# tooHotSpot/FGN

Hardware: AMD Instinct MI355X
Metric: query-imgs/sec (3-way 3-shot, 800x1333 FGN simple_test) (higher is better)
Workload: dtype f32; 1 GPU; cfg3: COCO2VOC 3-way 3-shot, query 3x800x1333, supports 9x3x256^2, ResNet-50-C4, R<=300 proposals, D<=100 detections, 1 episode(s) per GPU per step; h2d_in_step=True, gt_mask_rle_in_step=True, world_size_seen=1, phase_lock=rpn, caller_streams=2, support_cache=False, hip_graph=True, winograd_3x3=F(4x4,3x3)

## Files before the change

### fgn_amd/csrc/spatial.hip

```cpp
#include "common.h"

__global__ void nchw3_to_nhwc4_kernel(const float* __restrict__ x, float4* __restrict__ y, int HW,
                                      long long total) {
    for (long long i = blockIdx.x * (long long)blockDim.x + threadIdx.x; i < total;
         i += (long long)gridDim.x * blockDim.x) {
        const long long b = i / HW;
        const int p = (int)(i - b * HW);
        const float* s = x + b * 3 * HW + p;
        y[i] = make_float4(s[0], s[HW], s[2 * (size_t)HW], 0.f);
    }
}

extern "C" int fgn_nchw3_to_nhwc4_f32(const float* x, float* y, int n_img, int H, int W,
                                      hipStream_t stream) {
    if (!x || !y) return FGN_ERR_ARG;
    const long long total = (long long)n_img * H * W;
    if (total == 0) return FGN_OK;
    const int grid = (int)std::min<long long>((total + 255) / 256, 256 * 8);
    hipLaunchKernelGGL(nchw3_to_nhwc4_kernel, dim3(grid), dim3(256), 0, stream, x,
                       reinterpret_cast<float4*>(y), H * W, total);
    FGN_LAUNCH_CHECK();
    return FGN_OK;
}

// ... 155 lines not shown
    if (!src || !dst) return FGN_ERR_ARG;
    if (G < 0 || h < 0 || w < 0 || H < 0 || W < 0 || h > RESIZE_MAX_DIM || w > RESIZE_MAX_DIM || H > RESIZE_MAX_DIM ||
        W > RESIZE_MAX_DIM)
        return FGN_ERR_SHAPE;
    if ((long long)G * H * W == 0) return FGN_OK;
    if (h == 0 || w == 0) return FGN_ERR_SHAPE;
    const int chunks = cdiv(W + 3, 256);
    const long long units = (long long)G * H * chunks;
    if (units > INT32_MAX - 16 * RESIZE_GRID_CAP) return FGN_ERR_SHAPE;
    const int grid = (int)std::min<long long>((units + RESIZE_BLOCK / 64 - 1) / (RESIZE_BLOCK / 64), RESIZE_GRID_CAP * 4);
    hipLaunchKernelGGL(resize_mask_u8_kernel, dim3(grid), dim3(RESIZE_BLOCK), 0, stream, src, dst, h, w, H, W, chunks,
                       (int)units);
    FGN_LAUNCH_CHECK();
    return FGN_OK;
}

__global__ void maxpool3x3s2_kernel(const float4* __restrict__ x, float4* __restrict__ y, int H, int W,
                                    int C4, int Ho, int Wo, long long total) {
    for (long long i = blockIdx.x * (long long)blockDim.x + threadIdx.x; i < total;
         i += (long long)gridDim.x * blockDim.x) {
        const int c = (int)(i % C4);
        long long r = i / C4;
        const int ox = (int)(r % Wo);
        r /= Wo;
        const int oy = (int)(r % Ho);
        const long long b = r / Ho;
        float4 m = make_float4(-INFINITY, -INFINITY, -INFINITY, -INFINITY);
#pragma unroll
        for (int ky = 0; ky < 3; ++ky) {
            const int iy = oy * 2 - 1 + ky;
            if ((unsigned)iy >= (unsigned)H) continue;
#pragma unroll
            for (int kx = 0; kx < 3; ++kx) {
                const int ix = ox * 2 - 1 + kx;
                if ((unsigned)ix >= (unsigned)W) continue;
                const float4 v = x[((b * H + iy) * W + ix) * C4 + c];
                m.x = fmaxf(m.x, v.x); m.y = fmaxf(m.y, v.y);
                m.z = fmaxf(m.z, v.z); m.w = fmaxf(m.w, v.w);
            }
        }
        y[i] = m;
    }
}

extern "C" int fgn_maxpool3x3s2_nhwc_f32(const float* x, float* y, int n_img, int H, int W, int C,
                                         hipStream_t stream) {
    if (!x || !y) return FGN_ERR_ARG;
    if (C % 4) return FGN_ERR_SHAPE;
    const int Ho = (H + 2 - 3) / 2 + 1, Wo = (W + 2 - 3) / 2 + 1;
    const long long total = (long long)n_img * Ho * Wo * (C / 4);
    if (total == 0) return FGN_OK;
    const int grid = (int)std::min<long long>((total + 255) / 256, 256 * 16);
    hipLaunchKernelGGL(maxpool3x3s2_kernel, dim3(grid), dim3(256), 0, stream,
                       reinterpret_cast<const float4*>(x), reinterpret_cast<float4*>(y), H, W, C / 4, Ho,
                       Wo, total);
    FGN_LAUNCH_CHECK();
    return FGN_OK;
}

struct AxisSample {
    int lo, hi;
    float l, h;
    bool valid;
};

__device__ __forceinline__ AxisSample axis_sample(float c, int size) {
    AxisSample s;
    s.valid = !(c < -1.0f || c > (float)size);
    if (c <= 0.f) c = 0.f;
    int lo = (int)c;
    int hi;
    if (lo >= size - 1) {
        hi = lo = size - 1;
        c = (float)lo;
    } else {
        hi = lo + 1;
    }
    s.lo = lo; s.hi = hi;
    s.l = c - (float)lo;
    s.h = 1.f - s.l;
    return s;
}

__global__ __launch_bounds__(256) void roi_align_kernel(const float* __restrict__ fmap,
                                                        const float* __restrict__ rois,
                                                        float* __restrict__ out,
                                                        const int32_t* __restrict__ n_rois_dev, int n_rois,
                                                        int H, int W, int C, int P, float spatial_scale,
                                                        int sampling_ratio, int aligned,
                                                        const float* __restrict__ post_shift, int relu,
                                                        const float* __restrict__ fmap2, float* __restrict__ out2, int C2,
                                                        const float* __restrict__ post_shift2, int relu2) {
    const int bin = blockIdx.x;
    const int r = bin / (P * P);
    int nr = n_rois;
    if (n_rois_dev) nr = min(nr, *n_rois_dev);
    if (r >= nr) return;
    const int pb = bin - r * P * P;
    const int ph = pb / P, pw = pb - ph * P;

    const float* roi = rois + (size_t)r * 5;
    const int b = (int)roi[0];
    const float off = aligned ? 0.5f : 0.f;
    const float x1 = roi[1] * spatial_scale - off;
    const float y1 = roi[2] * spatial_scale - off;
    const float x2 = roi[3] * spatial_scale - off;
    const float y2 = roi[4] * spatial_scale - off;
    float rw = x2 - x1, rh = y2 - y1;
    if (!aligned) {
        rw = fmaxf(rw, 1.f);
        rh = fmaxf(rh, 1.f);
    }
    const float bin_h = rh / (float)P, bin_w = rw / (float)P;
    const int gh = sampling_ratio > 0 ? sampling_ratio : (int)ceilf(rh / (float)P);
    const int gw = sampling_ratio > 0 ? sampling_ratio : (int)ceilf(rw / (float)P);
    const float count = (float)max(gh * gw, 1);
    const float* base1 = fmap + (size_t)b * H * W * C;
    const float* base2 = fmap2 ? fmap2 + (size_t)b * H * W * C2 : nullptr;
    const int c_all = C + (fmap2 ? C2 : 0);
    const int C1 = C;

    constexpr int MAXS = 32;
    __shared__ float wy_sh[MAXS], wx_sh[MAXS];
    __shared__ int span_sh[4];
    if (threadIdx.x < 2) {
        const bool is_y = threadIdx.x == 0;
        const int g = is_y ? gh : gw, size = is_y ? H : W;
        const float start = (is_y ? y1 + (float)ph * bin_h : x1 + (float)pw * bin_w), step = is_y ? bin_h : bin_w;
        float* w = is_y ? wy_sh : wx_sh;
        int first = 0, last = -1;
        if (g > 0) {
            const AxisSample s0 = axis_sample(start + 0.5f * step / (float)g, size);
            const AxisSample s1 = axis_sample(start + ((float)(g - 1) + 0.5f) * step / (float)g, size);
            first = min(s0.lo, s1.lo);
            last = max(s0.hi, s1.hi);
        }
        const int n = last - first + 1;
        span_sh[is_y ? 0 : 2] = first;
        span_sh[is_y ? 1 : 3] = n;
        if (n <= MAXS) {
            for (int i = 0; i < n; ++i) w[i] = 0.f;
            for (int i = 0; i < g; ++i) {
                const AxisSample sp = axis_sample(start + ((float)i + 0.5f) * step / (float)g, size);
                if (sp.valid) {
                    w[sp.lo - first] += sp.h;
                    w[sp.hi - first] += sp.l;
                }
            }
        }
    }
    __syncthreads();
    const int y0 = span_sh[0], ny = span_sh[1], x0 = span_sh[2], nx = span_sh[3];
    const bool separable = ny <= MAXS && nx <= MAXS;

    for (int cc = threadIdx.x * 4; cc < c_all; cc += blockDim.x * 4) {
        const bool snd = cc >= C1;
        const float* base = snd ? base2 : base1;
        const int c = snd ? cc - C1 : cc;
        C = snd ? C2 : C1;
        if (snd) { out = out2; post_shift = post_shift2; relu = relu2; }
        float4 acc = make_float4(0.f, 0.f, 0.f, 0.f);
        if (separable) {
            for (int py = 0; py < ny; ++py) {
                const float wyv = wy_sh[py];
                const float* row = base + ((size_t)(y0 + py) * W + x0) * C + c;
                float4 racc = make_float4(0.f, 0.f, 0.f, 0.f);
                for (int px = 0; px < nx; ++px) {
                    const float wv = wx_sh[px];
                    const float4 v = *reinterpret_cast<const float4*>(row + (size_t)px * C);
                    racc.x += wv * v.x; racc.y += wv * v.y; racc.z += wv * v.z; racc.w += wv * v.w;
                }
                acc.x += wyv * racc.x; acc.y += wyv * racc.y; acc.z += wyv * racc.z; acc.w += wyv * racc.w;
            }
        } else {
            for (int iy = 0; iy < gh; ++iy) {
                const float y = y1 + (float)ph * bin_h + ((float)iy + 0.5f) * bin_h / (float)gh;
                const AxisSample sy = axis_sample(y, H);
                for (int ix = 0; ix < gw; ++ix) {
                    const float x = x1 + (float)pw * bin_w + ((float)ix + 0.5f) * bin_w / (float)gw;
                    const AxisSample sx = axis_sample(x, W);
                    if (!(sy.valid && sx.valid)) continue;
                    const float w1 = sy.h * sx.h, w2 = sy.h * sx.l, w3 = sy.l * sx.h, w4 = sy.l * sx.l;
                    const float4 v1 = *reinterpret_cast<const float4*>(base + ((size_t)sy.lo * W + sx.lo) * C + c);
                    const float4 v2 = *reinterpret_cast<const float4*>(base + ((size_t)sy.lo * W + sx.hi) * C + c);
                    const float4 v3 = *reinterpret_cast<const float4*>(base + ((size_t)sy.hi * W + sx.lo) * C + c);
                    const float4 v4 = *reinterpret_cast<const float4*>(base + ((size_t)sy.hi * W + sx.hi) * C + c);
                    acc.x += w1 * v1.x + w2 * v2.x + w3 * v3.x + w4 * v4.x;
                    acc.y += w1 * v1.y + w2 * v2.y + w3 * v3.y + w4 * v4.y;
                    acc.z += w1 * v1.z + w2 * v2.z + w3 * v3.z + w4 * v4.z;
                    acc.w += w1 * v1.w + w2 * v2.w + w3 * v3.w + w4 * v4.w;
                }
            }
        }
        acc.x /= count; acc.y /= count; acc.z /= count; acc.w /= count;
        if (post_shift) {
            const float4 sh = *reinterpret_cast<const float4*>(post_shift + c);
            acc.x += sh.x; acc.y += sh.y; acc.z += sh.z; acc.w += sh.w;
        }
        if (relu) {
            acc.x = fmaxf(acc.x, 0.f); acc.y = fmaxf(acc.y, 0.f); acc.z = fmaxf(acc.z, 0.f); acc.w = fmaxf(acc.w, 0.f);
        }
        *reinterpret_cast<float4*>(out + ((size_t)r * P * P + pb) * C + c) = acc;
    }
}

__global__ __launch_bounds__(256) void roi_align_mask_kernel(const uint8_t* __restrict__ mask,
                                                             const float* __restrict__ rois,
                                                             float* __restrict__ out, int n_rois, int H, int W,
                                                             int P, float spatial_scale, int sampling_ratio,
                                                             int aligned) {
    const int i = (blockIdx.x * blockDim.x + threadIdx.x) >> 6;
    const int lane = threadIdx.x & 63;
    if (i >= n_rois * P * P) return;
    const int r = i / (P * P);
    const int pb = i - r * P * P;
    const int ph = pb / P, pw = pb - ph * P;
    const float* roi = rois + (size_t)r * 5;
    const int b = (int)roi[0];
    const float off = aligned ? 0.5f : 0.f;
    const float x1 = roi[1] * spatial_scale - off;
    const float y1 = roi[2] * spatial_scale - off;
    const float x2 = roi[3] * spatial_scale - off;
    const float y2 = roi[4] * spatial_scale - off;
    float rw = x2 - x1, rh = y2 - y1;
    if (!aligned) {
        rw = fmaxf(rw, 1.f);
        rh = fmaxf(rh, 1.f);
    }
    const float bin_h = rh / (float)P, bin_w = rw / (float)P;
    const int gh = sampling_ratio > 0 ? sampling_ratio : (int)ceilf(rh / (float)P);
    const int gw = sampling_ratio > 0 ? sampling_ratio : (int)ceilf(rw / (float)P);
    const float count = (float)max(gh * gw, 1);
    const uint8_t* base = mask + (size_t)b * H * W;
    float acc = 0.f;
    for (int s = lane; s < gh * gw; s += 64) {
        const int iy = s / gw, ix = s - iy * gw;
        const float y = y1 + (float)ph * bin_h + ((float)iy + 0.5f) * bin_h / (float)gh;
        const float x = x1 + (float)pw * bin_w + ((float)ix + 0.5f) * bin_w / (float)gw;
        const AxisSample sy = axis_sample(y, H);
        const AxisSample sx = axis_sample(x, W);
        if (!(sy.valid && sx.valid)) continue;
        const float v1 = base[(size_t)sy.lo * W + sx.lo] ? 1.f : 0.f;
        const float v2 = base[(size_t)sy.lo * W + sx.hi] ? 1.f : 0.f;
        const float v3 = base[(size_t)sy.hi * W + sx.lo] ? 1.f : 0.f;
        const float v4 = base[(size_t)sy.hi * W + sx.hi] ? 1.f : 0.f;
        acc += sy.h * sx.h * v1 + sy.h * sx.l * v2 + sy.l * sx.h * v3 + sy.l * sx.l * v4;
    }
    acc = wave_reduce_sum(acc);
    if (lane == 0) out[i] = acc / count;
}

extern "C" int fgn_roi_align_nhwc_f32(const float* fmap, const float* rois, float* out,
                                      const int32_t* n_rois_dev, int n_rois, int n_img, int H, int W, int C,
                                      int out_size, float spatial_scale, int sampling_ratio, int aligned,
                                      const float* post_shift, int relu, hipStream_t stream) {
    if (!fmap || !rois || !out) return FGN_ERR_ARG;
    if (C % 4 || out_size <= 0) return FGN_ERR_SHAPE;
    (void)n_img;
    if (n_rois == 0) return FGN_OK;
    const int threads = C >= 1024 ? 256 : (C >= 512 ? 128 : 64);
    hipLaunchKernelGGL(roi_align_kernel, dim3(n_rois * out_size * out_size), dim3(threads), 0, stream, fmap,
                       rois, out, n_rois_dev, n_rois, H, W, C, out_size, spatial_scale, sampling_ratio,
                       aligned, post_shift, relu, (const float*)nullptr, (float*)nullptr, 0, (const float*)nullptr, 0);
    FGN_LAUNCH_CHECK();
    return FGN_OK;
}

extern "C" int fgn_roi_align2_nhwc_f32(const float* fmap, const float* fmap2, const float* rois, float* out, float* out2,
                                       const int32_t* n_rois_dev, int n_rois, int n_img, int H, int W, int C, int C2,
                                       int out_size, float spatial_scale, int sampling_ratio, int aligned,
                                       const float* post_shift2, int relu2, hipStream_t stream) {
    if (!fmap || !fmap2 || !rois || !out || !out2) return FGN_ERR_ARG;
    if (C % 4 || C2 % 4 || out_size <= 0) return FGN_ERR_SHAPE;
    (void)n_img;
    if (n_rois == 0) return FGN_OK;
    const int quads = (C + C2) / 4;
    const int threads = quads % 192 == 0 ? 192 : (quads >= 256 ? 256 : (quads >= 128 ? 128 : 64));
    hipLaunchKernelGGL(roi_align_kernel, dim3(n_rois * out_size * out_size), dim3(threads), 0, stream, fmap,
                       rois, out, n_rois_dev, n_rois, H, W, C, out_size, spatial_scale, sampling_ratio,
                       aligned, (const float*)nullptr, 0, fmap2, out2, C2, post_shift2, relu2);
    FGN_LAUNCH_CHECK();
    return FGN_OK;
}

extern "C" int fgn_roi_align_mask_u8(const uint8_t* mask, const float* rois, float* out, int n_rois, int n_img,
                                     int H, int W, int out_size, float spatial_scale, int sampling_ratio,
                                     int aligned, hipStream_t stream) {
    if (!mask || !rois || !out) return FGN_ERR_ARG;
    (void)n_img;
    if (n_rois == 0) return FGN_OK;
    const int total = n_rois * out_size * out_size;
    hipLaunchKernelGGL(roi_align_mask_kernel, dim3(cdiv(total, 4)), dim3(256), 0, stream, mask, rois, out,
                       n_rois, H, W, out_size, spatial_scale, sampling_ratio, aligned);
    FGN_LAUNCH_CHECK();
    return FGN_OK;
}

constexpr int CV_WAVES = 16;
__global__ __launch_bounds__(64 * CV_WAVES) void class_vector_kernel(const float* __restrict__ x,
                                                                     const float* __restrict__ w,
                                                                     float* __restrict__ out, int K, int P, int C) {
    __shared__ float4 part[CV_WAVES][64];
    const int g = blockIdx.x;
    const int c = (blockIdx.y * 64 + (threadIdx.x & 63)) * 4;
    const int wv = threadIdx.x >> 6;
    const int KP = K * P;
    float4 acc = make_float4(0.f, 0.f, 0.f, 0.f);
    if (c < C) {
        for (int i = wv; i < KP; i += CV_WAVES) {
            const float4 v = *reinterpret_cast<const float4*>(x + ((size_t)g * KP + i) * C + c);
            const float s = w ? w[(size_t)g * KP + i] : 1.f;
            acc.x += v.x * s; acc.y += v.y * s; acc.z += v.z * s; acc.w += v.w * s;
        }
    }
    part[wv][threadIdx.x & 63] = acc;
    __syncthreads();
    if (wv == 0 && c < C) {
        float4 o = make_float4(0.f, 0.f, 0.f, 0.f);
#pragma unroll
        for (int k = 0; k < CV_WAVES; ++k) {
            const float4 a = part[k][threadIdx.x];
            o.x += a.x; o.y += a.y; o.z += a.z; o.w += a.w;
        }
        const float inv = 1.f / (float)KP;
        o.x *= inv; o.y *= inv; o.z *= inv; o.w *= inv;
        *reinterpret_cast<float4*>(out + (size_t)g * C + c) = o;
    }
}

extern "C" int fgn_support_class_vectors_f32(const float* x, const float* weights, float* out, int n_groups,
                                             int K, int P, int C, hipStream_t stream) {
    if (!x || !out) return FGN_ERR_ARG;
    if (C % 4) return FGN_ERR_SHAPE;
    if (n_groups == 0) return FGN_OK;
    hipLaunchKernelGGL(class_vector_kernel, dim3(n_groups, cdiv(C, 256)), dim3(64 * CV_WAVES), 0, stream, x, weights,
                       out, K, P, C);
    FGN_LAUNCH_CHECK();
    return FGN_OK;
}

__global__ void kmean_kernel(const float4* __restrict__ x, float4* __restrict__ out, int K, long long PC4,
                             long long total) {
    const float inv = 1.f / (float)K;
    for (long long i = blockIdx.x * (long long)blockDim.x + threadIdx.x; i < total;
         i += (long long)gridDim.x * blockDim.x) {
        const long long g = i / PC4, r = i - g * PC4;
        float4 acc = make_float4(0.f, 0.f, 0.f, 0.f);
        for (int k = 0; k < K; ++k) {
            const float4 v = x[(g * K + k) * PC4 + r];
            acc.x += v.x; acc.y += v.y; acc.z += v.z; acc.w += v.w;
        }
        out[i] = make_float4(acc.x * inv, acc.y * inv, acc.z * inv, acc.w * inv);
    }
}

extern "C" int fgn_support_kmean_f32(const float* x, float* out, int n_groups, int K, int P, int C,
                                     hipStream_t stream) {
    if (!x || !out) return FGN_ERR_ARG;
    if (C % 4) return FGN_ERR_SHAPE;
    const long long pc4 = (long long)P * C / 4, total = pc4 * n_groups;
    if (total == 0) return FGN_OK;
    const int grid = (int)std::min<long long>((total + 255) / 256, 2048);
    hipLaunchKernelGGL(kmean_kernel, dim3(grid), dim3(256), 0, stream, reinterpret_cast<const float4*>(x),
// ... 54 lines not shown
```

### fgn_amd/detector.py

```python
from __future__ import annotations

import copy
import os
from collections import OrderedDict
from typing import Dict, List, NamedTuple, Optional, Union

import numpy as np
import torch

from . import config as _config
from . import ops, rle
from .weights import backbone_state_from_pretrained, init_state_dict


_R50_BLOCKS = (3, 4, 6, 3)


def normalise_config(n_ways, k_shots, backbone=None, rpn_head=None, roi_head=None, test_cfg=None,
                     train_cfg=None) -> dict:
    cfg = _config.fgn_r50_c4_config(n_ways, k_shots)
    if backbone:
        if 'stage_blocks' in backbone:
            cfg['backbone'].update(backbone)
        else:
# ... 1139 lines not shown
                    y1_all.record_stream(side)

        def support_tail():
            if msh:
                self._support_rois(sc, B, dev, x_all[:ns], None if y1_all is None else y1_all[:ns])
            else:
                self._support_back(sc, B, dev)
        qry_fmap = None
        if cached:
            sc = support_code
        elif merged:
            sc = self._support_front(spp_imgs, spp_bboxes, spp_isegmaps, B, dev, main, defer_backbone=True)
            qry_fmap, spp_fmaps = self.extract_feat_pair(qry, sc.pop('spp'), phase_counter)
            backbone_done = main.record_event()
            with torch.cuda.stream(side):
                side.wait_event(backbone_done)
                self._support_vectors(sc, spp_fmaps)
                vec_ready = side.record_event()
                support_tail()
            if side is not main and not torch.cuda.is_current_stream_capturing():
                spp_fmaps.record_stream(side)
        else:
            side.wait_stream(main)
            with torch.cuda.stream(side):
                sc = self._support_front(spp_imgs, spp_bboxes, spp_isegmaps, B, dev, side)
                vec_ready = side.record_event()
                support_tail()
        vec = sc['vec']

        if qry_fmap is None:
            qry_fmap = self.extract_feat(qry)
        fh, fw, C = qry_fmap.shape[1:]
        if tr is not None:
            tr['qry_fmap'], tr['spp_fmaps'] = qry_fmap, sc.get('spp_fmaps')

        if not cached:
            main.wait_event(vec_ready)
        rpn_start = main.record_event()
        self._phase_mark('rpn', phase_counter)
        if P['rpn_conv_wg'] is not None and ops.winograd_fits(B * N, fh, fw, C, P['rpn_conv_wg'].cout,
                                                              P['rpn_conv_wg'].m):
            x = ops.conv3x3_winograd(qry_fmap, P['rpn_conv_wg'], in_scale=vec, a_img_div=N)
        else:
            x = ops.conv2d(ops.scale_channels(qry_fmap, vec, N), P['rpn_conv'])
        self._phase_mark('rpn_conv', phase_counter)
        head = ops.conv2d(x, P['rpn_head'])
        A = P['anchors'].shape[0]
        logits, scores, deltas = ops.rpn_merge(head, B, N, A)

        g_map = None
        if not cached:
            with torch.cuda.stream(side):
                if P['sh0_lin'] is not None and side is not main:
                    side.wait_event(rpn_start)
                    g_map = ops.conv2d(qry_fmap, P['sh0_lin'])
                spp_ready = side.record_event()
            if not torch.cuda.is_current_stream_capturing():
                for key in ('spp_fmaps', 'vec', 'masks7') if msh else ('spp_fmaps', 'vec', 'S', 'cat_mean', 'cat_mean_mp', 'masks7'):
                    sc[key].record_stream(main)
                if g_map is not None:
                    g_map.record_stream(main)
                    qry_fmap.record_stream(side)
        ih, iw = int(img_shape[0][0]), int(img_shape[0][1])
        if any(int(s[0]) != ih or int(s[1]) != iw for s in img_shape):
            raise ValueError('all images of a batch must share img_shape (the dataset batches by size)')
        props, n_props, rois_all = ops.rpn_proposals(scores, deltas, P['anchors'], fh, fw, rp['anchor_stride'], ih, iw,
                                                     rp['target_means'], rp['target_stds'], tc['rpn']['nms_pre'],
                                                     tc['rpn']['min_bbox_size'], tc['rpn']['nms_iou_threshold'],
                                                     tc['rpn']['max_per_img'], with_rois=True)
        if not cached:
            main.wait_event(spp_ready)
        if tr is not None:
            tr.update(class_vec=vec, rpn_logits=logits, rpn_scores=scores, rpn_deltas=deltas, proposals=props,
                      n_props=n_props)

        self._phase_mark('proposals', phase_counter)
        rel, bh = rh['relation'], rh['bbox_head']
        R, D = props.shape[1], tc['rcnn']['max_per_img']
        cnt_all = n_props[0:1] if B == 1 else None
        if g_map is None and P['sh0_lin'] is not None:
            g_map = ops.conv2d(qry_fmap, P['sh0_lin'])
        if msh:
            inv = 1.0 / rh['featmap_stride']
            ops.roi_align(qry_fmap, rois_all, PS, inv, rh['roi_sampling_ratio'], True, cnt_all, out=x_all[ns:])
            if y1_all is not None:
                ops.roi_align(g_map, rois_all, PS, inv, rh['roi_sampling_ratio'], True, cnt_all,
                              post_shift=P['sh0_shift'], relu=True, out=y1_all[ns:])
            cnt_plus = None if cnt_all is None else cnt_all + ns
            feats_all = self._shared_head(x_all, cnt_plus, y1=y1_all)
            self._support_finish(sc, feats_all[:ns], B)
            feats = feats_all[ns:]
        else:
            _, feats = self._roi_feats(qry_fmap, g_map, rois_all, cnt_all)
        S, cat_mean, cat_mean_mp, masks7 = sc['S'], sc['cat_mean'], sc['cat_mean_mp'], sc['masks7']
        if tr is not None:
            tr.update(spp_masks7=masks7, spp_cat_mean=cat_mean, spp_cat_mean_mp=cat_mean_mp)
        Q = ops.conv2d(feats, P['rel_q'], n_img_dev=cnt_all)
        cls_raw, reg_raw = ops.relation_gn_head(Q, S, rois_all, P['gn_w'], P['gn_b'], P['fc_w'], P['fc_b'], N,
                                                rel['gn_groups'], rel['gn_eps'], cnt_all)
        rec = _ResultRecord(B, D, 2 * PS, dev)
        rec.clear_head()
        packed = self.use_packed_transfers
        det_all, lab_all, n_det_all, mrois_all = ops.det_post(
            rois_all, cls_raw, reg_raw, N, ih, iw, bh['target_means'], bh['target_stds'], tc['rcnn']['score_thr'],
            tc['rcnn']['nms_iou_threshold'], D, n_props, img_index=0, batch=B,
            out=(rec.det.view(B * D, 5), rec.lab.view(B * D), rec.cnt.view(B)))
        dets = [det_all[i * D:(i + 1) * D] for i in range(B)]
        labs = [lab_all[i * D:(i + 1) * D] for i in range(B)]
        n_dets = [n_det_all[i:i + 1] for i in range(B)]
        self._phase_mark('mask', phase_counter)
        nd_all = n_dets[0] if B == 1 else None
        vmask = ops.gather_support_vectors(cat_mean_mp, lab_all, mrois_all, N, nd_all)
        _, mf = self._roi_feats(qry_fmap, g_map, mrois_all, nd_all)
        mlog, mprob = self._mask_head(mf, vmask, nd_all, prob_out=rec.prob.view(B * D, 2 * PS, 2 * PS))
        outs = []
        for i in range(B):
            det, lab, n_det = dets[i], labs[i], n_dets[i]
            mp_i = mprob[i * D:(i + 1) * D]
            skip_empty = self._skip_empty()
            rle_bytes, rle_len, rle_ovf = ops.mask_rle(mp_i, det, ih, iw, tc['rcnn']['mask_thr_binary'], n_det,
                                                       skip_empty=skip_empty,
                                                       out=(rec.rle[i], rec.rle_len[i], rec.rle_ovf[i]))
            if tr is not None:
                masks = ops.mask_paste(mp_i, det, ih, iw, tc['rcnn']['mask_thr_binary'], n_det, skip_empty=skip_empty)
                tr.setdefault('per_image', []).append(dict(
                    rois=rois_all[i * R:(i + 1) * R], roi_feats=feats[i * R:(i + 1) * R], Q=Q[i * R:(i + 1) * R],
                    cls_raw=cls_raw[i * R * N:(i + 1) * R * N], reg_raw=reg_raw[i * R * N:(i + 1) * R * N],
                    det=det, lab=lab, n_det=n_det, mask_logits=mlog[i * D:(i + 1) * D], mask_prob=mp_i,
                    masks=masks, mask_feats=mf[i * D:(i + 1) * D]))
            outs.append(dict(det_bboxes=det, det_labels=lab, n_dets=n_det, mask_prob=mp_i, rle_bytes=rle_bytes,
                             rle_len=rle_len, rle_overflow=rle_ovf, img_hw=(ih, iw), record=rec if packed else None))
        return outs

    MAX_SLOTS = 64

    def _pinned_slot(self, batch: int, max_det: int, n_gt: int, mask_size: int = 14, n_ov: int = 0) -> dict:
        key = (batch, max_det, mask_size, ops.RLE_BYTE_CAP)
        ring = self._pinned.setdefault(key, [])
        slot = next((s for s in ring if not s['busy']), None)
        if slot is None:
            if len(ring) >= self.MAX_SLOTS:
                raise ops._lib.FgnHipError(f'{self.MAX_SLOTS} batches are in flight without pack_results(); '
                                           'pack (or drop and call release_results on) earlier detect_device outputs')
            rec = _ResultRecord(batch, max_det, mask_size, pinned=True)
            slot = dict(key=key, busy=False, gt_cap=0, rec=rec, det=rec.det, lab=rec.lab, cnt=rec.cnt, rle_len=rec.rle_len,
                        rle_ovf=rec.rle_ovf, rle=rec.rle, prob=rec.prob)
            ring.append(slot)
        if n_gt > slot['gt_cap']:
            cap = max(64, 2 * n_gt)
            slot.update(gt_cap=cap, gt_buf=torch.empty(cap * (ops.RLE_BYTE_CAP + 8), dtype=torch.uint8, pin_memory=True))
        if n_ov > slot.get('ov_cap', 0):
            cap = max(64, 2 * n_ov)
            slot.update(ov_cap=cap, ov_buf=torch.empty(cap * (max_det + 1) + batch * max_det, dtype=torch.int32,
                                                       pin_memory=True))
        slot['busy'] = True
        return slot

    @staticmethod
    def release_results(dets: list) -> None:
        if dets and 'host' in dets[0]:
            dets[0]['host']['busy'] = False

    def _start_download(self, outs: list, main, also_wait=None) -> None:
        cp = self._stream_for('copy', main)
        max_det = outs[0]['det_bboxes'].shape[0]
        n_gt = sum(d['gt_rle'][1].shape[0] for d in outs if 'gt_rle' in d)
        rec = outs[0].get('record')
        n_ov = sum(d['gt_rle'][1].shape[0] for d in outs if 'overlap' in d)
        slot = self._pinned_slot(len(outs), max_det, n_gt, outs[0]['mask_prob'].shape[-1], n_ov)
        cp.wait_stream(main)
# ... 108 lines not shown
```

### fgn_amd/ops.py

```python
from __future__ import annotations

import ctypes as C
import math
import os
from dataclasses import dataclass
from typing import Optional

import numpy as np
import torch

from . import lib as _lib


PROFILE = None

FUSED_SHORTCUT = os.environ.get('FGN_FUSED_SHORTCUT', '1') != '0'
GEMM_MATH = os.environ.get('FGN_GEMM_MATH', 'h2')
X3_KERNELS = {64: 'conv_pw_x3_kernel<2, 1, 6, 2, true>', 128: 'conv_pw_x3_kernel<2, 2, 6, 2, true>'}
H2_KERNELS = {64: 'conv_pw_h2_kernel<2, 2, 1, 2, %s>', 128: 'conv_pw_h2_kernel<2, 2, 2, 2, %s>', 264: 'conv_pw_h2_kernel<4, 1, 1, 2, %s>'}


def x3_kernel(rows: int, cout: int, k: int, grp_rows: int = 0, grp_valid: int = 0) -> str:
    return X3_KERNELS.get(_lib.load().fgn_x3_row_tile(rows, cout, k, grp_rows, grp_valid), 'conv_pw_x3_kernel<?>')

# ... 906 lines not shown
    if h == 0 or w == 0:
        raise _lib.FgnHipError('resize_masks: empty source masks')
    _lib.check(_lib.load().fgn_resize_mask_u8(_ptr(masks), _ptr(out), g, h, w, H, W, _stream()), 'fgn_resize_mask_u8')
    return out


def maxpool3x3s2(x: torch.Tensor, out: Optional[torch.Tensor] = None) -> torch.Tensor:
    _chk(x, 'x')
    n, h, w, c = x.shape
    shape = (n, (h - 1) // 2 + 1, (w - 1) // 2 + 1, c)
    if out is None:
        y = torch.empty(shape, device=x.device, dtype=torch.float32)
    else:
        _chk(out, 'out')
        if tuple(out.shape) != shape:
            raise _lib.FgnHipError('maxpool3x3s2: bad out shape')
        y = out
    _lib.check(_lib.load().fgn_maxpool3x3s2_nhwc_f32(_ptr(x), _ptr(y), n, h, w, c, _stream()),
               'fgn_maxpool3x3s2_nhwc_f32')
    return y


def group_norm(x: torch.Tensor, gamma: torch.Tensor, beta: torch.Tensor, groups: int, eps: float = 1e-5,
               relu: bool = False, residual: Optional[torch.Tensor] = None, inplace: bool = False) -> torch.Tensor:
    _chk(x, 'x')
    _chk(gamma, 'gamma')
    _chk(beta, 'beta')
    n, h, w, c = x.shape
    if gamma.numel() != c or beta.numel() != c or c % groups != 0:
        raise _lib.FgnHipError('group_norm: bad gamma/beta/groups')
    if residual is not None:
        _chk(residual, 'residual')
        if residual.shape != x.shape:
            raise _lib.FgnHipError('group_norm: bad residual shape')
    lib = _lib.load()
    nbytes = lib.fgn_group_norm_workspace_bytes(n, h * w, c, groups)
    ws = torch.empty(max(nbytes // 8, 1), device=x.device, dtype=torch.float64)
    y = x if inplace else torch.empty_like(x)
    _lib.check(lib.fgn_group_norm_nhwc_f32(_ptr(x), _ptr(y), _ptr(gamma), _ptr(beta), _ptr(residual), _ptr(ws), nbytes,
                                           n, h * w, c, groups, float(eps), int(relu), _stream()),
               'fgn_group_norm_nhwc_f32')
    return y


def avgpool2x2(x: torch.Tensor) -> torch.Tensor:
    _chk(x, 'x')
    n, h, w, c = x.shape
    y = torch.empty((n, (h + 1) // 2, (w + 1) // 2, c), device=x.device, dtype=torch.float32)
    _lib.check(_lib.load().fgn_avgpool2x2_nhwc_f32(_ptr(x), _ptr(y), n, h, w, c, _stream()), 'fgn_avgpool2x2_nhwc_f32')
    return y


def roi_align(fmap: torch.Tensor, rois: torch.Tensor, out_size: int, spatial_scale: float,
              sampling_ratio: int, aligned: bool, n_rois_dev: Optional[torch.Tensor] = None,
              post_shift: Optional[torch.Tensor] = None, relu: bool = False,
              out: Optional[torch.Tensor] = None) -> torch.Tensor:
    _chk(fmap, 'fmap')
    _chk(rois, 'rois')
    b, h, w, c = fmap.shape
    if post_shift is not None:
        _chk(post_shift, 'post_shift')
        if post_shift.numel() != c:
            raise _lib.FgnHipError('roi_align: post_shift must be [C]')
    if rois.dim() != 2 or rois.shape[1] != 5:
        raise _lib.FgnHipError('roi_align: rois must be [R,5]')
    r = rois.shape[0]
    if out is None:
        out = torch.empty((r, out_size, out_size, c), device=fmap.device, dtype=torch.float32)
    else:
        _chk(out, 'out')
        if tuple(out.shape) != (r, out_size, out_size, c):
            raise _lib.FgnHipError('roi_align: bad out shape')
    if n_rois_dev is not None:
        _chk(n_rois_dev, 'n_rois_dev', torch.int32)
    rc = _lib.load().fgn_roi_align_nhwc_f32(_ptr(fmap), _ptr(rois), _ptr(out), _ptr(n_rois_dev), r, b, h, w, c,
                                            out_size, float(spatial_scale), sampling_ratio, int(aligned),
                                            _ptr(post_shift), int(relu), _stream())
    _lib.check(rc, 'fgn_roi_align_nhwc_f32')
    return out


def roi_align2(fmap: torch.Tensor, fmap2: torch.Tensor, rois: torch.Tensor, out_size: int, spatial_scale: float,
               sampling_ratio: int, aligned: bool, n_rois_dev: Optional[torch.Tensor] = None,
               post_shift2: Optional[torch.Tensor] = None, relu2: bool = False):
    _chk(fmap, 'fmap')
    _chk(fmap2, 'fmap2')
    _chk(rois, 'rois')
    b, h, w, c = fmap.shape
    c2 = fmap2.shape[3]
    if tuple(fmap2.shape[:3]) != (b, h, w) or rois.dim() != 2 or rois.shape[1] != 5:
        raise _lib.FgnHipError('roi_align2: operand shapes inconsistent')
    if post_shift2 is not None:
        _chk(post_shift2, 'post_shift2')
        if post_shift2.numel() != c2:
            raise _lib.FgnHipError('roi_align2: post_shift2 must be [C2]')
    if n_rois_dev is not None:
        _chk(n_rois_dev, 'n_rois_dev', torch.int32)
    r = rois.shape[0]
    out = torch.empty((r, out_size, out_size, c), device=fmap.device, dtype=torch.float32)
    out2 = torch.empty((r, out_size, out_size, c2), device=fmap.device, dtype=torch.float32)
    rc = _lib.load().fgn_roi_align2_nhwc_f32(_ptr(fmap), _ptr(fmap2), _ptr(rois), _ptr(out), _ptr(out2), _ptr(n_rois_dev),
                                             r, b, h, w, c, c2, out_size, float(spatial_scale), sampling_ratio,
                                             int(aligned), _ptr(post_shift2), int(relu2), _stream())
    _lib.check(rc, 'fgn_roi_align2_nhwc_f32')
    return out, out2


def roi_align_mask(mask_u8: torch.Tensor, rois: torch.Tensor, out_size: int, spatial_scale: float,
                   sampling_ratio: int, aligned: bool) -> torch.Tensor:
    _chk(mask_u8, 'mask', torch.uint8)
    _chk(rois, 'rois')
    b, h, w = mask_u8.shape
    r = rois.shape[0]
    out = torch.empty((r, out_size, out_size), device=mask_u8.device, dtype=torch.float32)
    rc = _lib.load().fgn_roi_align_mask_u8(_ptr(mask_u8), _ptr(rois), _ptr(out), r, b, h, w, out_size,
                                           float(spatial_scale), sampling_ratio, int(aligned), _stream())
    _lib.check(rc, 'fgn_roi_align_mask_u8')
    return out


def support_class_vectors(x: torch.Tensor, weights: Optional[torch.Tensor], n_groups: int, k: int) -> torch.Tensor:
    _chk(x, 'x')
    c = x.shape[-1]
    p = x[0].numel() // c
    if x.shape[0] != n_groups * k:
        raise _lib.FgnHipError('support_class_vectors: leading dim != n_groups*k')
    if weights is not None:
        _chk(weights, 'weights')
        if weights.numel() != n_groups * k * p:
            raise _lib.FgnHipError('support_class_vectors: weights shape mismatch')
    out = torch.empty((n_groups, c), device=x.device, dtype=torch.float32)
    rc = _lib.load().fgn_support_class_vectors_f32(_ptr(x), _ptr(weights), _ptr(out), n_groups, k, p, c, _stream())
    _lib.check(rc, 'fgn_support_class_vectors_f32')
    return out


def scale_channels(x: torch.Tensor, v: torch.Tensor, div: int) -> torch.Tensor:
    _chk(x, 'x')
    _chk(v, 'v')
    n_out, c = v.shape
    if x.shape[0] * div != n_out or x.shape[-1] != c:
        raise _lib.FgnHipError('scale_channels: operand shapes inconsistent')
    out = torch.empty((n_out,) + tuple(x.shape[1:]), device=x.device, dtype=torch.float32)
    p = math.prod(x.shape[1:-1])
    _lib.check(_lib.load().fgn_scale_channels_f32(_ptr(x), _ptr(v), _ptr(out), n_out, div, p, c, _stream()),
               'fgn_scale_channels_f32')
    return out


def support_kmean(x: torch.Tensor, n_groups: int, k: int) -> torch.Tensor:
    _chk(x, 'x')
    if x.shape[0] != n_groups * k:
        raise _lib.FgnHipError('support_kmean: leading dim != n_groups*k')
    c = x.shape[-1]
    p = x[0].numel() // c
    out = torch.empty((n_groups,) + tuple(x.shape[1:]), device=x.device, dtype=torch.float32)
    rc = _lib.load().fgn_support_kmean_f32(_ptr(x), _ptr(out), n_groups, k, p, c, _stream())
    _lib.check(rc, 'fgn_support_kmean_f32')
    return out


def gather_support_vectors(table: torch.Tensor, labels: torch.Tensor, rois: Optional[torch.Tensor],
                           n_ways: int, n_dev: Optional[torch.Tensor] = None) -> torch.Tensor:
    _chk(table, 'table')
    _chk(labels, 'labels', torch.int64)
    n, c = labels.shape[0], table.shape[-1]
    if rois is not None:
        _chk(rois, 'rois')
        if rois.shape[0] < n or rois.shape[1] != 5:
            raise _lib.FgnHipError('gather_support_vectors: rois must be [>=n,5]')
    out = zeros((n, c), table.device)
    rc = _lib.load().fgn_gather_support_vectors_f32(_ptr(table), _ptr(labels), _ptr(rois), _ptr(out), _ptr(n_dev),
                                                    n, n_ways, c, _stream())
    _lib.check(rc, 'fgn_gather_support_vectors_f32')
    return out


def relation_gn_head(q: torch.Tensor, s: torch.Tensor, rois: torch.Tensor, gn_w, gn_b, fc_w, fc_b,
                     n_ways: int, gn_groups: int, eps: float, n_rois_dev: Optional[torch.Tensor] = None,
                     rel_out: Optional[torch.Tensor] = None):
    for t, nm in ((q, 'Q'), (s, 'S'), (rois, 'rois'), (gn_w, 'gn_w'), (gn_b, 'gn_b'), (fc_w, 'fc_w'), (fc_b, 'fc_b')):
        _chk(t, nm)
    r, p, _, c = q.shape
# ... 567 lines not shown
```

Measured before the change: 320.8 img/s.

## Fuse dual RoIAlign calls and compute bilinear weights with wave lane broadcasts

In the query path, the two separate roi_align launches over the query feature map and g_map are replaced by one roi_align2 launch that writes into the preallocated outputs. Inside the kernel, the per-axis interpolation weights are now computed in parallel, one slot per lane, and broadcast with readlane instead of being built serially by two threads into shared memory behind a __syncthreads. A templated Q processes several channel quads per thread, and the block shape is chosen so the thread count times Q matches the quad count. The aim is to cut launch count, the serial weight setup and barrier latency, and to raise memory-level parallelism per thread. In exchange it adds register pressure and relies on wave64 lane indexing.

```diff
diff --git a/fgn_amd/csrc/spatial.hip b/fgn_amd/csrc/spatial.hip
--- a/fgn_amd/csrc/spatial.hip
+++ b/fgn_amd/csrc/spatial.hip
@@ -261,19 +261,53 @@
     return s;
 }
 
-__global__ __launch_bounds__(256) void roi_align_kernel(const float* __restrict__ fmap,
-                                                        const float* __restrict__ rois,
-                                                        float* __restrict__ out,
-                                                        const int32_t* __restrict__ n_rois_dev, int n_rois,
-                                                        int H, int W, int C, int P, float spatial_scale,
-                                                        int sampling_ratio, int aligned,
-                                                        const float* __restrict__ post_shift, int relu,
-                                                        const float* __restrict__ fmap2, float* __restrict__ out2, int C2,
-                                                        const float* __restrict__ post_shift2, int relu2) {
+constexpr int ROI_MAXS = 32;
+constexpr int ROI_MAX_THREADS = 256;
+constexpr int ROI_MAX_Q = 4;
+
+__device__ __forceinline__ float roi_lane_f(float v, int lane) {
+    return __int_as_float(__builtin_amdgcn_readlane(__float_as_int(v), lane));
+}
+
+__device__ __forceinline__ void roi_add_sample(float& w, const AxisSample& sp, int first, int slot) {
+    if (sp.valid) {
+        if (sp.lo - first == slot) w += sp.h;
+        if (sp.hi - first == slot) w += sp.l;
+    }
+}
+
+__device__ __forceinline__ void roi_finish(float4 a, float count, float inv_count, bool count_pow2, const float* shift,
+                                           int relu, int c, float* dst) {
+    if (count_pow2) {
+        a.x *= inv_count; a.y *= inv_count; a.z *= inv_count; a.w *= inv_count;
+    } else {
+        a.x /= count; a.y /= count; a.z /= count; a.w /= count;
+    }
+    if (shift) {
+        const float4 sh = *reinterpret_cast<const float4*>(shift + c);
+        a.x += sh.x; a.y += sh.y; a.z += sh.z; a.w += sh.w;
+    }
+    if (relu) {
+        a.x = fmaxf(a.x, 0.f); a.y = fmaxf(a.y, 0.f); a.z = fmaxf(a.z, 0.f); a.w = fmaxf(a.w, 0.f);
+    }
+    *reinterpret_cast<float4*>(dst + c) = a;
+}
+
+template <int Q>
+__global__ __launch_bounds__(ROI_MAX_THREADS) void roi_align_kernel(const float* __restrict__ fmap,
+                                                                    const float* __restrict__ rois,
+                                                                    float* __restrict__ out,
+                                                                    const int32_t* __restrict__ n_rois_dev, int n_rois,
+                                                                    int H, int W, int C, int P, float spatial_scale,
+                                                                    int sampling_ratio, int aligned,
+                                                                    const float* __restrict__ post_shift, int relu,
+                                                                    const float* __restrict__ fmap2,
+                                                                    float* __restrict__ out2, int C2,
+                                                                    const float* __restrict__ post_shift2, int relu2) {
+    int nr = n_rois;
+    if (n_rois_dev) nr = min(nr, *n_rois_dev);
     const int bin = blockIdx.x;
     const int r = bin / (P * P);
-    int nr = n_rois;
-    if (n_rois_dev) nr = min(nr, *n_rois_dev);
     if (r >= nr) return;
     const int pb = bin - r * P * P;
     const int ph = pb / P, pw = pb - ph * P;
@@ -293,65 +327,46 @@
     const float bin_h = rh / (float)P, bin_w = rw / (float)P;
     const int gh = sampling_ratio > 0 ? sampling_ratio : (int)ceilf(rh / (float)P);
     const int gw = sampling_ratio > 0 ? sampling_ratio : (int)ceilf(rw / (float)P);
-    const float count = (float)max(gh * gw, 1);
+    const int cnt = max(gh * gw, 1);
+    const float count = (float)cnt, inv_count = 1.f / count;
+    const bool count_pow2 = (cnt & (cnt - 1)) == 0;
     const float* base1 = fmap + (size_t)b * H * W * C;
-    const float* base2 = fmap2 ? fmap2 + (size_t)b * H * W * C2 : nullptr;
-    const int c_all = C + (fmap2 ? C2 : 0);
-    const int C1 = C;
-
-    constexpr int MAXS = 32;
-    __shared__ float wy_sh[MAXS], wx_sh[MAXS];
-    __shared__ int span_sh[4];
-    if (threadIdx.x < 2) {
-        const bool is_y = threadIdx.x == 0;
-        const int g = is_y ? gh : gw, size = is_y ? H : W;
-        const float start = (is_y ? y1 + (float)ph * bin_h : x1 + (float)pw * bin_w), step = is_y ? bin_h : bin_w;
-        float* w = is_y ? wy_sh : wx_sh;
-        int first = 0, last = -1;
-        if (g > 0) {
-            const AxisSample s0 = axis_sample(start + 0.5f * step / (float)g, size);
-            const AxisSample s1 = axis_sample(start + ((float)(g - 1) + 0.5f) * step / (float)g, size);
-            first = min(s0.lo, s1.lo);
-            last = max(s0.hi, s1.hi);
-        }
-        const int n = last - first + 1;
-        span_sh[is_y ? 0 : 2] = first;
-        span_sh[is_y ? 1 : 3] = n;
-        if (n <= MAXS) {
-            for (int i = 0; i < n; ++i) w[i] = 0.f;
-            for (int i = 0; i < g; ++i) {
-                const AxisSample sp = axis_sample(start + ((float)i + 0.5f) * step / (float)g, size);
-                if (sp.valid) {
-                    w[sp.lo - first] += sp.h;
-                    w[sp.hi - first] += sp.l;
-                }
-            }
-        }
-    }
-    __syncthreads();
-    const int y0 = span_sh[0], ny = span_sh[1], x0 = span_sh[2], nx = span_sh[3];
-    const bool separable = ny <= MAXS && nx <= MAXS;
-
-    for (int cc = threadIdx.x * 4; cc < c_all; cc += blockDim.x * 4) {
-        const bool snd = cc >= C1;
-        const float* base = snd ? base2 : base1;
-        const int c = snd ? cc - C1 : cc;
-        C = snd ? C2 : C1;
-        if (snd) { out = out2; post_shift = post_shift2; relu = relu2; }
-        float4 acc = make_float4(0.f, 0.f, 0.f, 0.f);
-        if (separable) {
-            for (int py = 0; py < ny; ++py) {
-                const float wyv = wy_sh[py];
-                const float* row = base + ((size_t)(y0 + py) * W + x0) * C + c;
-                float4 racc = make_float4(0.f, 0.f, 0.f, 0.f);
-                for (int px = 0; px < nx; ++px) {
-                    const float wv = wx_sh[px];
-                    const float4 v = *reinterpret_cast<const float4*>(row + (size_t)px * C);
-                    racc.x += wv * v.x; racc.y += wv * v.y; racc.z += wv * v.z; racc.w += wv * v.w;
-                }
-                acc.x += wyv * racc.x; acc.y += wyv * racc.y; acc.z += wyv * racc.z; acc.w += wyv * racc.w;
-            }
-        } else {
+    const float* base2 = (fmap2 ? fmap2 : fmap) + (size_t)b * H * W * C2;
+    const int quads1 = C >> 2;
+    const int quads = quads1 + (fmap2 ? C2 >> 2 : 0);
+
+    const int lane = threadIdx.x & 63;
+    const bool is_y = lane < ROI_MAXS;
+    const int slot = lane & (ROI_MAXS - 1);
+    const int g = is_y ? gh : gw, size = is_y ? H : W;
+    const float start = (is_y ? y1 + (float)ph * bin_h : x1 + (float)pw * bin_w), step = is_y ? bin_h : bin_w;
+    int first = 0, last = -1;
+    AxisSample s0 = {}, s1 = {};
+    if (g > 0) {
+        s0 = axis_sample(start + 0.5f * step / (float)g, size);
+        s1 = g > 1 ? axis_sample(start + ((float)(g - 1) + 0.5f) * step / (float)g, size) : s0;
+        first = min(s0.lo, s1.lo);
+        last = max(s0.hi, s1.hi);
+    }
+    const int n = last - first + 1;
+    float wgt = 0.f;
+    if (g > 0 && n <= ROI_MAXS) {
+        roi_add_sample(wgt, s0, first, slot);
+        for (int i = 1; i < g - 1; ++i)
+            roi_add_sample(wgt, axis_sample(start + ((float)i + 0.5f) * step / (float)g, size), first, slot);
+        if (g > 1) roi_add_sample(wgt, s1, first, slot);
+    }
+    const int y0 = __builtin_amdgcn_readlane(first, 0), ny = __builtin_amdgcn_readlane(n, 0);
+    const int x0 = __builtin_amdgcn_readlane(first, ROI_MAXS), nx = __builtin_amdgcn_readlane(n, ROI_MAXS);
+    const bool separable = ny <= ROI_MAXS && nx <= ROI_MAXS;
+
+    if (!separable) {
+        for (int q = threadIdx.x; q < quads; q += blockDim.x) {
+            const bool snd = q >= quads1;
+            const int c = (snd ? q - quads1 : q) * 4;
+            const size_t Cq = snd ? C2 : C;
+            const float* base = (snd ? base2 : base1) + c;
+            float4 acc = make_float4(0.f, 0.f, 0.f, 0.f);
             for (int iy = 0; iy < gh; ++iy) {
                 const float y = y1 + (float)ph * bin_h + ((float)iy + 0.5f) * bin_h / (float)gh;
                 const AxisSample sy = axis_sample(y, H);
@@ -360,27 +375,99 @@
                     const AxisSample sx = axis_sample(x, W);
                     if (!(sy.valid && sx.valid)) continue;
                     const float w1 = sy.h * sx.h, w2 = sy.h * sx.l, w3 = sy.l * sx.h, w4 = sy.l * sx.l;
-                    const float4 v1 = *reinterpret_cast<const float4*>(base + ((size_t)sy.lo * W + sx.lo) * C + c);
-                    const float4 v2 = *reinterpret_cast<const float4*>(base + ((size_t)sy.lo * W + sx.hi) * C + c);
-                    const float4 v3 = *reinterpret_cast<const float4*>(base + ((size_t)sy.hi * W + sx.lo) * C + c);
-                    const float4 v4 = *reinterpret_cast<const float4*>(base + ((size_t)sy.hi * W + sx.hi) * C + c);
+                    const float4 v1 = *reinterpret_cast<const float4*>(base + ((size_t)sy.lo * W + sx.lo) * Cq);
+                    const float4 v2 = *reinterpret_cast<const float4*>(base + ((size_t)sy.lo * W + sx.hi) * Cq);
+                    const float4 v3 = *reinterpret_cast<const float4*>(base + ((size_t)sy.hi * W + sx.lo) * Cq);
+                    const float4 v4 = *reinterpret_cast<const float4*>(base + ((size_t)sy.hi * W + sx.hi) * Cq);
                     acc.x += w1 * v1.x + w2 * v2.x + w3 * v3.x + w4 * v4.x;
                     acc.y += w1 * v1.y + w2 * v2.y + w3 * v3.y + w4 * v4.y;
                     acc.z += w1 * v1.z + w2 * v2.z + w3 * v3.z + w4 * v4.z;
                     acc.w += w1 * v1.w + w2 * v2.w + w3 * v3.w + w4 * v4.w;
                 }
             }
-        }
-        acc.x /= count; acc.y /= count; acc.z /= count; acc.w /= count;
-        if (post_shift) {
-            const float4 sh = *reinterpret_cast<const float4*>(post_shift + c);
-            acc.x += sh.x; acc.y += sh.y; acc.z += sh.z; acc.w += sh.w;
-        }
-        if (relu) {
-            acc.x = fmaxf(acc.x, 0.f); acc.y = fmaxf(acc.y, 0.f); acc.z = fmaxf(acc.z, 0.f); acc.w = fmaxf(acc.w, 0.f);
-        }
-        *reinterpret_cast<float4*>(out + ((size_t)r * P * P + pb) * C + c) = acc;
-    }
+            roi_finish(acc, count, inv_count, count_pow2, snd ? post_shift2 : post_shift, snd ? relu2 : relu, c,
+                       (snd ? out2 : out) + ((size_t)r * P * P + pb) * Cq);
+        }
+        return;
+    }
+
+    for (int q0 = threadIdx.x; q0 < quads; q0 += blockDim.x * Q) {
+        const float* src[Q];
+        int pitch[Q], ch[Q];
+        bool on[Q], snd[Q];
+#pragma unroll
+        for (int k = 0; k < Q; ++k) {
+            int q = q0 + k * (int)blockDim.x;
+            on[k] = q < quads;
+            if (!on[k]) q = q0;
+            snd[k] = q >= quads1;
+            ch[k] = (snd[k] ? q - quads1 : q) * 4;
+            pitch[k] = snd[k] ? C2 : C;
+            src[k] = (snd[k] ? base2 : base1) + ch[k];
+        }
+        float4 acc[Q];
+#pragma unroll
+        for (int k = 0; k < Q; ++k) acc[k] = make_float4(0.f, 0.f, 0.f, 0.f);
+        for (int py = 0; py < ny; ++py) {
+            const float wyv = roi_lane_f(wgt, py);
+            const size_t pix = (size_t)(y0 + py) * W + x0;
+            const float* row[Q];
+            float4 racc[Q];
+#pragma unroll
+            for (int k = 0; k < Q; ++k) {
+                row[k] = src[k] + pix * pitch[k];
+                racc[k] = make_float4(0.f, 0.f, 0.f, 0.f);
+            }
+            for (int px = 0; px < nx; ++px) {
+                const float wv = roi_lane_f(wgt, ROI_MAXS + px);
+#pragma unroll
+                for (int k = 0; k < Q; ++k) {
+                    const float4 v = *reinterpret_cast<const float4*>(row[k]);
+                    row[k] += pitch[k];
+                    racc[k].x += wv * v.x; racc[k].y += wv * v.y; racc[k].z += wv * v.z; racc[k].w += wv * v.w;
+                }
+            }
+#pragma unroll
+            for (int k = 0; k < Q; ++k) {
+                acc[k].x += wyv * racc[k].x; acc[k].y += wyv * racc[k].y;
+                acc[k].z += wyv * racc[k].z; acc[k].w += wyv * racc[k].w;
+            }
+        }
+#pragma unroll
+        for (int k = 0; k < Q; ++k)
+            if (on[k])
+                roi_finish(acc[k], count, inv_count, count_pow2, snd[k] ? post_shift2 : post_shift, snd[k] ? relu2 : relu,
+                           ch[k], (snd[k] ? out2 : out) + ((size_t)r * P * P + pb) * pitch[k]);
+    }
+}
+
+static void roi_block_shape(int quads, int* threads, int* q) {
+    const int pref[] = {128, 192, 256, 64};
+    for (int t : pref)
+        for (int k = 1; k <= ROI_MAX_Q; ++k)
+            if (t * k == quads) { *threads = t; *q = k; return; }
+    *q = std::max(1, std::min(ROI_MAX_Q, cdiv(quads, 256)));
+    *threads = std::max(64, std::min(256, cdiv(cdiv(quads, *q), 64) * 64));
+}
+
+static void roi_launch(const float* fmap, const float* rois, float* out, const int32_t* n_rois_dev, int n_rois, int H,
+                       int W, int C, int out_size, float spatial_scale, int sampling_ratio, int aligned,
+                       const float* post_shift, int relu, const float* fmap2, float* out2, int C2,
+                       const float* post_shift2, int relu2, hipStream_t stream) {
+    int threads, q;
+    roi_block_shape((C + (fmap2 ? C2 : 0)) / 4, &threads, &q);
+    const dim3 grid(n_rois * out_size * out_size), block(threads);
+#define ROI_LAUNCH(Q)                                                                                                  \
+    hipLaunchKernelGGL(roi_align_kernel<Q>, grid, block, 0, stream, fmap, rois, out, n_rois_dev, n_rois, H, W, C,      \
+                       out_size, spatial_scale, sampling_ratio, aligned, post_shift, relu, fmap2, out2, C2,            \
+                       post_shift2, relu2)
+    switch (q) {
+        case 1: ROI_LAUNCH(1); break;
+        case 2: ROI_LAUNCH(2); break;
+        case 3: ROI_LAUNCH(3); break;
+        default: ROI_LAUNCH(4); break;
+    }
+#undef ROI_LAUNCH
 }
 
 __global__ __launch_bounds__(256) void roi_align_mask_kernel(const uint8_t* __restrict__ mask,
@@ -437,10 +524,8 @@
     if (C % 4 || out_size <= 0) return FGN_ERR_SHAPE;
     (void)n_img;
     if (n_rois == 0) return FGN_OK;
-    const int threads = C >= 1024 ? 256 : (C >= 512 ? 128 : 64);
-    hipLaunchKernelGGL(roi_align_kernel, dim3(n_rois * out_size * out_size), dim3(threads), 0, stream, fmap,
-                       rois, out, n_rois_dev, n_rois, H, W, C, out_size, spatial_scale, sampling_ratio,
-                       aligned, post_shift, relu, (const float*)nullptr, (float*)nullptr, 0, (const float*)nullptr, 0);
+    roi_launch(fmap, rois, out, n_rois_dev, n_rois, H, W, C, out_size, spatial_scale, sampling_ratio, aligned,
+               post_shift, relu, nullptr, nullptr, 0, nullptr, 0, stream);
     FGN_LAUNCH_CHECK();
     return FGN_OK;
 }
@@ -453,11 +538,8 @@
     if (C % 4 || C2 % 4 || out_size <= 0) return FGN_ERR_SHAPE;
     (void)n_img;
     if (n_rois == 0) return FGN_OK;
-    const int quads = (C + C2) / 4;
-    const int threads = quads % 192 == 0 ? 192 : (quads >= 256 ? 256 : (quads >= 128 ? 128 : 64));
-    hipLaunchKernelGGL(roi_align_kernel, dim3(n_rois * out_size * out_size), dim3(threads), 0, stream, fmap,
-                       rois, out, n_rois_dev, n_rois, H, W, C, out_size, spatial_scale, sampling_ratio,
-                       aligned, (const float*)nullptr, 0, fmap2, out2, C2, post_shift2, relu2);
+    roi_launch(fmap, rois, out, n_rois_dev, n_rois, H, W, C, out_size, spatial_scale, sampling_ratio, aligned, nullptr, 0,
+               fmap2, out2, C2, post_shift2, relu2, stream);
     FGN_LAUNCH_CHECK();
     return FGN_OK;
 }
diff --git a/fgn_amd/detector.py b/fgn_amd/detector.py
--- a/fgn_amd/detector.py
+++ b/fgn_amd/detector.py
@@ -1245,10 +1245,11 @@
             g_map = ops.conv2d(qry_fmap, P['sh0_lin'])
         if msh:
             inv = 1.0 / rh['featmap_stride']
-            ops.roi_align(qry_fmap, rois_all, PS, inv, rh['roi_sampling_ratio'], True, cnt_all, out=x_all[ns:])
             if y1_all is not None:
-                ops.roi_align(g_map, rois_all, PS, inv, rh['roi_sampling_ratio'], True, cnt_all,
-                              post_shift=P['sh0_shift'], relu=True, out=y1_all[ns:])
+                ops.roi_align2(qry_fmap, g_map, rois_all, PS, inv, rh['roi_sampling_ratio'], True, cnt_all,
+                               post_shift2=P['sh0_shift'], relu2=True, out=x_all[ns:], out2=y1_all[ns:])
+            else:
+                ops.roi_align(qry_fmap, rois_all, PS, inv, rh['roi_sampling_ratio'], True, cnt_all, out=x_all[ns:])
             cnt_plus = None if cnt_all is None else cnt_all + ns
             feats_all = self._shared_head(x_all, cnt_plus, y1=y1_all)
             self._support_finish(sc, feats_all[:ns], B)
diff --git a/fgn_amd/ops.py b/fgn_amd/ops.py
--- a/fgn_amd/ops.py
+++ b/fgn_amd/ops.py
@@ -1012,7 +1012,8 @@
 
 def roi_align2(fmap: torch.Tensor, fmap2: torch.Tensor, rois: torch.Tensor, out_size: int, spatial_scale: float,
                sampling_ratio: int, aligned: bool, n_rois_dev: Optional[torch.Tensor] = None,
-               post_shift2: Optional[torch.Tensor] = None, relu2: bool = False):
+               post_shift2: Optional[torch.Tensor] = None, relu2: bool = False,
+               out: Optional[torch.Tensor] = None, out2: Optional[torch.Tensor] = None):
     _chk(fmap, 'fmap')
     _chk(fmap2, 'fmap2')
     _chk(rois, 'rois')
@@ -1027,8 +1028,16 @@
     if n_rois_dev is not None:
         _chk(n_rois_dev, 'n_rois_dev', torch.int32)
     r = rois.shape[0]
-    out = torch.empty((r, out_size, out_size, c), device=fmap.device, dtype=torch.float32)
-    out2 = torch.empty((r, out_size, out_size, c2), device=fmap.device, dtype=torch.float32)
+    outs = []
+    for t, name, ch in ((out, 'out', c), (out2, 'out2', c2)):
+        if t is None:
+            t = torch.empty((r, out_size, out_size, ch), device=fmap.device, dtype=torch.float32)
+        else:
+            _chk(t, name)
+            if tuple(t.shape) != (r, out_size, out_size, ch):
+                raise _lib.FgnHipError(f'roi_align2: bad {name} shape')
+        outs.append(t)
+    out, out2 = outs
     rc = _lib.load().fgn_roi_align2_nhwc_f32(_ptr(fmap), _ptr(fmap2), _ptr(rois), _ptr(out), _ptr(out2), _ptr(n_rois_dev),
                                              r, b, h, w, c, c2, out_size, float(spatial_scale), sampling_ratio,
                                              int(aligned), _ptr(post_shift2), int(relu2), _stream())
```

After: 321.7 img/s (median of 6 runs). Within noise of the previous version (+0.3%).
